# kubernetes-sigs/karpenter

Hardware: AMD Instinct MI355X
Metric: pods scheduled/sec (Solve()) (higher is better)
Workload: dtype int64

## Files before the change

### karpenter_amd/csrc/fast_engine.h

```cpp
#pragma once
#include <type_traits>
#include "kernels.h"
#include "pdq_emul.h"

namespace ks {

constexpr int kFastRows = 4;
constexpr uint32_t kFastFree = 0xFFFFFFFFu;
constexpr uint32_t kFastLastBit = 0x80000000u;
constexpr int kFastEnt = 1024;
constexpr int kFastPool = 256;
constexpr int kFastMaxPareto = 16;
constexpr int kFastMaxVar = 12;
constexpr uint64_t kFastExtBit = 1ull << 63;
constexpr int kFastVarBits = 56;

struct FastClaim { uint64_t vmask; int32_t req[4]; };
template <int R> struct FastRec { uint64_t vmask; int32_t req[4]; uint64_t acc[R]; };
struct FastSlot { uint64_t cvmask; uint64_t dmask; int32_t size[4]; uint32_t tmplok; uint32_t kdef; };
struct FastEnt { uint64_t vmask; int32_t cap[4]; uint32_t info; uint32_t pad; };

struct FastPlan {
  int total_bytes, cap;
  int off_state, off_key, off_ord, off_snap, off_ent, off_pool, off_slot, off_misc, off_hot;
// ... 177 lines not shown
KS_FN KS_LDS T* fast_uniform(KS_LDS T* p) {
  return (KS_LDS T*)(uintptr_t)(uint32_t)__builtin_amdgcn_readfirstlane((int)(uint32_t)(uintptr_t)p);
}
#endif
template <class T>
KS_FN T* fast_uniform(T* p) {
#if KS_DEVICE
  const uint64_t u = (uint64_t)p;
  const uint32_t lo = (uint32_t)__builtin_amdgcn_readfirstlane((int)(uint32_t)u), hi = (uint32_t)__builtin_amdgcn_readfirstlane((int)(uint32_t)(u >> 32));
  return (T*)((uint64_t)lo | ((uint64_t)hi << 32));
#else
  return p;
#endif
}

template <bool H, int R> KS_FN ClaimRecs<H, R> fast_uniform(ClaimRecs<H, R> c) { c.p = fast_uniform(c.p); return c; }

#define KS_LIKELY(x) __builtin_expect(!!(x), 1)
#define KS_UNLIKELY(x) __builtin_expect(!!(x), 0)
#if KS_DEVICE
#define KS_COLD __device__ __attribute__((noinline))
#else
#define KS_COLD inline
#endif

KS_FN uint32_t fast_hash(uint64_t vm) {
  const uint32_t lo = (uint32_t)vm, hi = (uint32_t)(vm >> 32);
  return (((lo ^ ((hi << 15) | (hi >> 17))) * 0x9E3779B1u) >> 22) & (kFastEnt - 1);
}
KS_FN int fast_lookup(const KS_LDS FastEnt* ent, uint64_t vm, FastEnt& out) {
  uint32_t h = fast_hash(vm);
  for (int probe = 0; probe < kFastEnt; ++probe) {
    out = lds_get(&ent[h]);
    if (!(out.info & 1u)) return -1;
    if ((out.vmask & ~kFastExtBit) == vm) return (int)h;
    h = (h + 1) & (kFastEnt - 1);
  }
  return -1;
}
KS_FN bool fast_fits_first(const FastEnt& e, const int32_t* req, const int32_t* size) {
  return (int)(size[0] <= e.cap[0] - req[0]) & (int)(size[1] <= e.cap[1] - req[1]) & (int)(size[2] <= e.cap[2] - req[2]) & (int)(size[3] <= e.cap[3] - req[3]);
}
KS_FN bool fast_fits(const KS_LDS int32_t* pool, const FastEnt& e, const int32_t* req, const int32_t* size) {
  if (fast_fits_first(e, req, size)) return true;
  const int extra = (int)((e.info >> 8) & 0xFFu);
  const int off = (int)(e.info >> 16);
// ... 936 lines not shown
      const KS_LDS FastEnt* en = ent;
      W::for_n(n, [&](int i) { const uint32_t c = oo[i]; go[i] = c; gn[c] = ok_[i]; });
      W::for_n(n, [&](int c) {
        const FastClaim st = ls.state((uint32_t)c);
        FastEnt e;
        gs[c] = st;
        ge[c] = (uint16_t)fast_lookup(en, st.vmask, e);
      });
      W::store(S.n_claims_out, n_claims);
    }
    FastNodes nd{};
    if (F.nodes) nd = *F.nodes;
    if (status == 0 && nd.limit_hit) status = 2;
    if (status) W::store(S.status_out, status);
    Counters c{};
    c.bin_evaluations = n_tests + n_cold_tests + nd.n_tests; c.full_evaluations = n_steps; c.queue_pops = steps + nd.n_placed; c.sorts = steps; c.slow_sorts = order.slow_sorts;
    c.column_resets = (unsigned long long)n_evict; c.ref_bin_evaluations = n_ref + n_ref_extra + nd.n_ref;
    c.decline = (unsigned long long)(bail_code > 0 ? bail_code : 0);
    if (tc) for (int i = 0; i < 16; ++i) c.cycles[i] = tc[i];
#ifdef KSOLVE_PHASE_TIMERS
    for (int i = 0; i < 4; ++i) c.cycles[16 + i] = hs->hw[i];
    c.cycles[20] = t_small | (n_small << 44);
    c.cycles[18] = (hs->hw[2] << 32) | (unsigned long long)(hs->mail.simd[0] | (hs->mail.simd[1] << 8) | (hs->mail.simd[2] << 16) | (hs->mail.simd[3] << 24));
#endif
    if (F.nodes) c.cycles[19] = (unsigned long long)nd.variant;
    if (F.lim) c.full_filters = (unsigned long long)(F.lim->n_ids - (uint32_t)Pk->n_templates) | ((unsigned long long)R << 16) | ((unsigned long long)F.lim->first_claim << 32);
    if (W::leader()) *S.counters = c;
    W::sync();
  }
};

template <int GS, int R>
struct FastHotCtx {
  typename FastMem<GS, R>::o16 okey, oord; typename FastMem<GS, R>::States cst; KS_LDS FastEnt* ent; KS_LDS int32_t* pool;
  KS_LDS FastSlot* aslot; KS_LDS FastHot* hs;
};
enum { FEV_DONE = 0, FEV_REFRESH = 1, FEV_SLOT = 2, FEV_SLOWSORT = 3, FEV_PLACE = 4, FEV_NEWCLAIM = 5, FEV_COUNT = 6, FEV_SLOW = 7, FEV_CONT = 8, FEV_DEAD = 9 };

template <int R>
struct FastHelperK {
  LaneVar<uint32_t> tok[R];
  LaneVar<uint64_t> cvm[R], dm[R], gd[R];
  LaneVar<int32_t> z0[R], z1[R], z2[R], z3[R];
  uint32_t gen = 0xFFFFFFFFu, miss = 0;
};
template <class W, int R>
// ... 82 lines not shown
KS_DEV void fast_helper_run(const FastWork* f, char* lds) {
  const FastPlan& pl = f->plan;
  FastHotCtx<GS, R> cx;
  cx.hs = fast_uniform((KS_LDS FastHot*)(lds + pl.off_hot));
  cx.cst.p = fast_uniform((KS_LDS FastRec<R>*)(lds + pl.off_state));
  cx.okey = nullptr; cx.oord = nullptr;
  cx.ent = fast_uniform((KS_LDS FastEnt*)(lds + pl.off_ent));
  cx.pool = fast_uniform((KS_LDS int32_t*)(lds + pl.off_pool));
  cx.aslot = fast_uniform((KS_LDS FastSlot*)(lds + pl.off_slot));
  KS_LDS FastMail* const mail = &cx.hs->mail;
  FastHelperK<R> k;
  uint32_t seen = 0;
  for (;;) {
    const uint32_t w0 = mail_load(&mail->word[0]), w1 = mail_load(&mail->word[1]), quit = mail_load(&mail->quit);
    if (fast_uniform((int)quit) != 0) break;
    const uint32_t nxt = seen + 1u;
    const uint32_t w = (uint32_t)fast_uniform((int)((nxt & 1u) ? w1 : w0));
    if ((w >> 16) != (nxt & 0xFFFFu)) continue;
    fast_helper_serve<W, GS, R>(k, cx, nxt, w);
    seen = nxt;
  }
}
#endif

template <class W, int GS, int R>
KS_COLD int fast_slow_run(FastHotCtx<GS, R> cx, int budget) {
  budget = fast_uniform(budget);
  typedef typename FastMem<GS, R>::o16 o16;
  const unsigned long long t_in = W::clock();
  const o16 okey = fast_uniform(cx.okey), oord = fast_uniform(cx.oord);
  const typename FastMem<GS, R>::States cst = fast_uniform(cx.cst);
  KS_LDS FastEnt* const ent = fast_uniform(cx.ent);
  KS_LDS int32_t* const pool = fast_uniform(cx.pool);
  KS_LDS FastSlot* const aslot = fast_uniform(cx.aslot);
  KS_LDS FastHot* const hs = fast_uniform(cx.hs);
  const int np = fast_uniform(hs->np), max_steps_in = fast_uniform(hs->max_steps);
  const int max_steps = max_steps_in < 0 ? 0x7FFFFFFF : max_steps_in;
  const KS_GLOBAL uint32_t* const gqcls = (const KS_GLOBAL uint32_t*)fast_uniform(hs->q_class);
  const volatile int* const cancel = fast_uniform(hs->cancel);
  KS_GLOBAL uint32_t* const gqclaim = (KS_GLOBAL uint32_t*)fast_uniform(hs->q_claim);
  KS_GLOBAL uint32_t* const gqcnt = (KS_GLOBAL uint32_t*)fast_uniform(hs->q_cnt);
  int base = fast_uniform(hs->base), bi = fast_uniform(hs->bi), bn = fast_uniform(hs->bn), n = fast_uniform(hs->n), steps = fast_uniform(hs->steps), status = fast_uniform(hs->status);
  int pend_a = fast_uniform(hs->pend_a), pend_x = fast_uniform(hs->pend_x); uint32_t pend_mv = (uint32_t)fast_uniform((int)hs->pend_mv); bool pend_new = fast_uniform(hs->pend_new) != 0;
  unsigned long long n_steps = W::uniform(hs->n_steps), n_ref = W::uniform(hs->n_ref);
  LaneVar<uint32_t> cur[R], scls[R], tok[R], nxt_cls, bcls, oclaim, ocnt;
  LaneVar<uint64_t> cvm[R], dm[R], gd[R];
// ... 23 lines not shown
      if (bn > 0) {
        const int dn = bn, b0 = base;
        W::each([&](int l) { if (l < dn) { gqclaim[b0 + l] = oclaim.at(l); gqcnt[b0 + l] = ocnt.at(l); } });
        base += 64;
      }
      if (base >= np || status) { bn = 0; bi = 0; break; }
      bn = np - base < 64 ? np - base : 64;
      bi = 0;
      const int nb = base + 64;
      W::each([&](int l) { bcls.at(l) = nxt_cls.at(l); });
      W::each([&](int l) { if (nb + l < np) nxt_cls.at(l) = gqcls[nb + l]; });
      if ((base & 1023) == 0 && cancel) {
        const int cv = fast_uniform((int)W::poll_flag(cancel));
        if (cv > 0 || (cv < 0 && base >= -cv)) { status = 2; bn = 0; break; }
      }
    }
    if (KS_UNLIKELY(steps >= max_steps)) { status = 2; break; }
    if (KS_UNLIKELY(pend_a >= 0)) {
      if (pend_new) { ev = FEV_PLACE; break; }
      const int a = pend_a;
      if (!(a + 1 >= n || (uint32_t)okey[a + 1 < n ? a + 1 : a] >= pend_mv) &&
          !(n <= 12 || (n >= 50 && !fast_sampled(n, a)))) { ev = FEV_SLOWSORT; ev_arg = a; break; }
      pend_a = -1;
      int from = a;
      const uint32_t mv = pend_mv;
      for (;;) {
        LaneVar<uint32_t> kv, ov;
        const uint64_t less = W::ballot([&](int l) {
          const int i = from + 1 + l;
          if (i >= n) return false;
          const uint32_t k = okey[i];
          kv.at(l) = k; ov.at(l) = oord[i];
          return k < mv;
        });
        const int s_ = less == ~0ull ? 64 : ctz64(~less);
        if (s_ == 0) break;
        W::each([&](int l) { if (l < s_) { okey[from + l] = (uint16_t)kv.at(l); oord[from + l] = (uint16_t)ov.at(l); } });
        from += s_;
        if (s_ < 64) break;
      }
      if (from != a) {
        if (W::leader()) { okey[from] = (uint16_t)mv; oord[from] = (uint16_t)pend_x; }
        W::sync();
        const int b = from;
        W::each([&](int l) {
#pragma unroll
          for (int j = 0; j < R; ++j) { const uint32_t r = cur[j].at(l); cur[j].at(l) = r - (uint32_t)(((uint32_t)a < r && r <= (uint32_t)b) ? 1 : 0); }
        });
      }
    }
    KS_SEC(ts0)
    const uint32_t clsw = bcls.bcast(bi), kcls = clsw & ~kFastLastBit;
    int row = -1, sl = 0;
    if constexpr (R == 1) {
      const uint64_t m0 = W::ballot([&](int l) { return scls[0].at(l) == kcls; });
      if (KS_LIKELY(m0 != 0)) { row = 0; sl = ctz64(m0); }
    } else {
#pragma unroll
      for (int j = 0; j < R; ++j) {
        const uint64_t mj = W::ballot([&](int l) { return scls[j].at(l) == kcls; });
        if (mj != 0 && row < 0) { row = j; sl = ctz64(mj); }
      }
    }
    if (KS_UNLIKELY(row < 0)) { ev = FEV_SLOT; ev_arg = (int)kcls; break; }
    if constexpr (R == 1) row = 0;
    const int slot = row * 64 + sl;
    const FastSlot cs = lds_get(&aslot[slot]);
// ... 139 lines not shown
      cst.put_state((uint32_t)x, ns);
#pragma unroll
      for (int j = 0; j < R; ++j) cst.put_acc((uint32_t)x, j, accw[j]);
      if (s_ <= 0) okey[a] = (uint16_t)mvn;
      else { okey[a + s_] = (uint16_t)mvn; oord[a + s_] = (uint16_t)x; }
    }
    W::sync();
    KS_SEC(ts3)
    bi++; steps++;
    if (KS_UNLIKELY(cold_refresh)) { ev = FEV_REFRESH; ev_arg = x; break; }
    if (--budget <= 0 && pend_a < 0) { ev = FEV_CONT; break; }
  }
  if (ev == FEV_DONE && bn > 0) {
    const int dn = bi < bn ? bi : bn, b0 = base;
    W::each([&](int l) { if (l < dn) { gqclaim[b0 + l] = oclaim.at(l); gqcnt[b0 + l] = ocnt.at(l); } });
    bn = 0; bi = 0;
  }
  if (W::leader()) {
    hs->base = base; hs->bi = bi; hs->bn = bn; hs->n = n; hs->steps = steps; hs->status = status;
    hs->pend_a = pend_a; hs->pend_x = pend_x; hs->pend_mv = pend_mv; hs->pend_new = pend_new ? 1 : 0;
    hs->n_steps = n_steps; hs->n_ref = n_ref; hs->ev_arg = ev_arg;
    hs->hot_cycles += W::clock() - t_in;
#ifdef KSOLVE_PHASE_TIMERS
    hs->tsec[0] += ts0; hs->tsec[1] += ts1; hs->tsec[2] += ts2; hs->tsec[3] += ts3; hs->tsec[4] += ts4; hs->tsec[5] += ts5; hs->tsec[6] += ts6; hs->tsec[7] += ts7;
#endif
  }
#undef KS_SEC
  W::each([&](int l) {
#pragma unroll
    for (int j = 0; j < R; ++j) { hs->cur[j][l] = cur[j].at(l); hs->scls[j][l] = scls[j].at(l); }
    hs->nxt_cls[l] = nxt_cls.at(l); hs->bcls[l] = bcls.at(l); hs->oclaim[l] = oclaim.at(l); hs->ocnt[l] = ocnt.at(l);
  });
  W::sync();
  return ev;
}

template <class W, int GS, int R, bool HP = false>
KS_COLD int fast_hot_run(FastHotCtx<GS, R> cx) {
  typedef typename FastMem<GS, R>::o16 o16;
  KS_LDS FastHot* const hs = fast_uniform(cx.hs);
  if (fast_uniform(hs->pend_a) >= 0 || fast_uniform(hs->max_steps) >= 0 || fast_uniform(hs->status) != 0 || fast_uniform(hs->n) <= 0) return FEV_SLOW;
  const o16 okey = fast_uniform(cx.okey), oord = fast_uniform(cx.oord);
  const typename FastMem<GS, R>::States cst = fast_uniform(cx.cst);
  KS_LDS FastEnt* const ent = fast_uniform(cx.ent);
  KS_LDS int32_t* const pool = fast_uniform(cx.pool);
  KS_LDS FastSlot* const aslot = fast_uniform(cx.aslot);
  const int np = fast_uniform(hs->np), n = fast_uniform(hs->n);
  const KS_GLOBAL uint32_t* const gqcls = (const KS_GLOBAL uint32_t*)fast_uniform(hs->q_class);
  const bool polled = fast_uniform(hs->cancel) != nullptr;
  KS_GLOBAL uint32_t* const gqclaim = (KS_GLOBAL uint32_t*)fast_uniform(hs->q_claim);
  KS_GLOBAL uint32_t* const gqcnt = (KS_GLOBAL uint32_t*)fast_uniform(hs->q_cnt);
  int base = fast_uniform(hs->base), bi = fast_uniform(hs->bi), bn = fast_uniform(hs->bn), steps = fast_uniform(hs->steps);
  unsigned long long n_ref = W::uniform(hs->n_ref);
  const int bi_in = bi, base_in = base;
  LaneVar<uint32_t> cur[R], scls[R], tok[R], nxt_cls, bcls, oclaim, ocnt;
  LaneVar<uint64_t> cvm[R], dm[R], gd[R];
  LaneVar<int32_t> z0[R], z1[R], z2[R], z3[R];
  W::each([&](int l) {
#pragma unroll
    for (int j = 0; j < R; ++j) {
      cur[j].at(l) = hs->cur[j][l]; scls[j].at(l) = hs->scls[j][l];
      if constexpr (!HP) {
        const FastSlot s = lds_get(&aslot[j * 64 + l]);
// ... 67 lines not shown
  auto stage_a = [&](int i) {
    clsw = bcls.bcast(i & 63);
    const uint32_t kcls = clsw & ~kFastLastBit;
    row = 0;
    if constexpr (R == 1) {
      const uint64_t m0 = W::ballot([&](int l) { return scls[0].at(l) == kcls; });
      slbitA = m0 & (0ull - m0);
      sl = ctz64(m0 | (1ull << 63));
    } else {
      uint64_t mf = 0;
#pragma unroll
      for (int j = R - 1; j >= 0; --j) {
        const uint64_t mj = W::ballot([&](int l) { return scls[j].at(l) == kcls; });
        row = mj != 0 ? j : row; mf = mj != 0 ? mj : mf;
      }
      slbitA = mf & (0ull - mf);
      sl = ctz64(mf | (1ull << 63));
    }
    rc0 = cur[0].bcast(sl);
#pragma unroll
    for (int j = 1; j < R; ++j) { const uint32_t cj = cur[j].bcast(sl); rc0 = row == j ? cj : rc0; }
    order_reads(rc0);
  };
  for (;;) {
    const int bf = bn - ((base + bn >= np || (polled && ((base + 64) & 1023) == 0)) ? 1 : 0);
    if (bi < bf) { stage_a(bi); read_done(); gather(); }
    int bfx = bf;
    while (bi < bfx) {
      uint64_t bad = 0;
      const int slot = row * 64 + sl;
      const FastSlot cs = lds_get(&aslot[slot]);
      const uint64_t slbit = slbitA;
      const int rws = row;
      uint64_t vm = 0;
      auto select = [&]() {
        const int rem = n - (int)rc0;
        vm = rem >= 64 ? ~0ull : ((1ull << (rem < 0 ? 0 : rem)) - 1ull);
        return W::ballot([&](int l) { return (awv.at(l) & slbit) != 0; }) & vm;
      };
      uint64_t okm = select();
      if constexpr (HP) {
        const int x0 = (int)xv.bcast(ctz64(okm | (1ull << 63)));
        if (KS_UNLIKELY((okm != 0) & ((x0 == pend1) | (x0 == pend2)))) {
          const uint32_t dn = (uint32_t)fast_uniform((int)dwl.bcast(0)) >> 1;
          const bool stale1 = pend1 >= 0 && (int32_t)(dn - seq) < 0, stale2 = pend2 >= 0 && (int32_t)(dn - (seq - 1u)) < 0;
          if ((x0 == pend1 && stale1) || (x0 == pend2 && stale2)) {
#ifdef KSOLVE_PHASE_TIMERS
            const unsigned long long tw0 = W::clock();
#endif
            const uint32_t c1 = (uint32_t)(pend1 < 0 ? 0 : pend1), c2 = (uint32_t)(pend2 < 0 ? 0 : pend2);
            uint64_t a1 = 0, a2 = 0;
            uint32_t dw2 = 0;
#if KS_DEVICE
            for (uint32_t spins = 0;; ++spins) {
              const uint32_t dv = mail_load(&mail->done);
              W::order();
              const uint64_t v1 = cst.acc(c1, 0), v2 = cst.acc(c2, 0);
              dw2 = (uint32_t)fast_uniform((int)dv); a1 = W::uniform(v1); a2 = W::uniform(v2);
              if ((int32_t)((dw2 >> 1) - seq) >= 0) break;
              if (spins > (1u << 22)) { dead = true; break; }
// ... 28 lines not shown
#pragma unroll
          for (int j = 0; j < 4; ++j) {
            const int rj = r + 64 * j;
            m4[j] = W::ballot([&](int l) { return ((cst.acc(x4[j].at(l), rws) & slbit) != 0) & (rj + l < n); });
          }
          n_ext++;
#pragma unroll
          for (int j = 3; j >= 0; --j) found = m4[j] != 0 ? r + 64 * j : found;
          r += 256;
        }
        if (found >= 0) {
          rc0 = (uint32_t)found;
          order_reads(rc0);
          gather();
          okm = select();
        }
      }
      const int first_ok = ctz64(okm | (1ull << 63));
      const int a = (int)rc0 + first_ok;
      const int x = (int)xv.bcast(first_ok);
      const uint32_t cnt = kv.bcast(first_ok);
      bad |= cnt >= 65534u ? ~0ull : 0ull;
      FastClaim ns;
      LaneVar<uint64_t> nmv; LaneVar<int32_t> n0v, n1v, n2v, n3v;
      W::each([&](int l) {
        nmv.at(l) = mvv.at(l) & cs.cvmask;
        n0v.at(l) = q0.at(l) + cs.size[0]; n1v.at(l) = q1.at(l) + cs.size[1]; n2v.at(l) = q2.at(l) + cs.size[2]; n3v.at(l) = q3.at(l) + cs.size[3];
      });
      ns.vmask = nmv.bcast(first_ok);
      ns.req[0] = n0v.bcast(first_ok); ns.req[1] = n1v.bcast(first_ok); ns.req[2] = n2v.bcast(first_ok); ns.req[3] = n3v.bcast(first_ok);
      const uint32_t mvn = cnt + 1;
      const uint64_t lessm = W::ballot([&](int l) { return kv.at(l) < mvn; }) & vm;
      const uint64_t tsh = (lessm >> 1) >> first_ok;
      const int sm = ctz64(~tsh);
      bad |= first_ok + 1 + sm >= 64 ? ~0ull : 0ull;
      {
        const uint32_t d1 = (uint32_t)a - e1, d2 = (uint32_t)a - e2, d3 = (uint32_t)a - e3;
        const uint32_t dmin = fast_umin_s(fast_umin_s(d1, d2), d3);
        bad |= ((sm != 0) & (inexact_b | (dmin <= 2u))) ? ~0ull : 0ull;
      }
      if (KS_UNLIKELY(bad != 0)) { bfx = bi; continue; }
      if constexpr (HP) {
        static_assert(!HP || R == 1, "the two-wavefront loop: one row of class slots");
        {
          const uint32_t dw = (uint32_t)fast_uniform((int)dwl.bcast(0));
          if (KS_UNLIKELY(((int32_t)((dw >> 1) - (seq - 1u)) < 0) | ((dw & 1u) != 0))) {
            const uint32_t dw2 = wait_for(seq - 1u);
#ifdef KSOLVE_PHASE_TIMERS
            hw2++;
#endif
            if ((dw2 & 1u) | (uint32_t)dead) break;
          }
        }
        ++seq;
        const int fo = first_ok; const uint32_t sq = seq;
        W::each([&](int l) {
          if (l == fo) {
            FastClaim mine;
            mine.vmask = nmv.at(l); mine.req[0] = n0v.at(l); mine.req[1] = n1v.at(l); mine.req[2] = n2v.at(l); mine.req[3] = n3v.at(l);
            cst.put_state(xv.at(l), mine);
            W::order();
            mail_store(&mail->word[sq & 1u], (sq << 16) | xv.at(l));
          }
        });
        pend2 = pend1; pend1 = x;
#ifdef KSOLVE_PHASE_TIMERS
        t_post = W::clock();
#endif
#if !KS_DEVICE
        if (fast_emu_helper_eager()) wait_for(seq);
#endif
        {
          const int rb = (int)rc0, smv = sm;
          W::each([&](int l) {
            if (l >= fo && l <= fo + smv) {
              const bool me = l == fo;
              const int dst = me ? rb + l + smv : rb + l - 1;
              okey[dst] = (uint16_t)(me ? kv.at(l) + 1u : kv.at(l)); oord[dst] = (uint16_t)xv.at(l);
            }
          });
        }
        W::order();
// ... 36 lines not shown
            okey[dst] = (uint16_t)(me ? kv.at(l) + 1u : kv.at(l)); oord[dst] = (uint16_t)xv.at(l);
          }
        });
      }
      {
        const uint32_t ua1 = (uint32_t)a + 1u, su = (uint32_t)sm;
        const uint32_t lastm = (uint32_t)((int32_t)clsw >> 31);
        const int bb = bi;
        W::each([&](int l) {
          const bool mine = l == bb;
          oclaim.at(l) = mine ? (uint32_t)x : oclaim.at(l); ocnt.at(l) = mine ? cnt : ocnt.at(l);
#pragma unroll
          for (int j = 0; j < R; ++j) {
            const bool me = j * 64 + l == slot;
            const uint32_t fm = me ? lastm : 0u;
            const uint32_t rr = cur[j].at(l);
            cur[j].at(l) = me ? (uint32_t)a : rr - (uint32_t)((rr - ua1) < su);
            scls[j].at(l) |= fm; tok[j].at(l) &= ~fm;
          }
        });
      }
      n_ref += (unsigned long long)((uint32_t)a + 1u);
      const uint32_t tbit = 1u << (uint32_t)(ns.vmask >> 56);
      LaneVar<uint64_t> mlv[R], evm[R];
      LaneVar<int32_t> c0[R], c1[R], c2[R], c3[R];
      uint64_t rowm[R];
      if constexpr (R > 1) {
        W::each([&](int l) {
#pragma unroll
          for (int j = 0; j < R; ++j) mlv[j].at(l) = ns.vmask & cvm[j].at(l);
        });
#pragma unroll
        for (int j = 0; j < R; ++j)
          rowm[j] = W::ballot([&](int l) { return (tok[j].at(l) & tbit) != 0; }) &
                    W::ballot([&](int l) { return (((mlv[j].at(l) & dm[j].at(l)) + dm[j].at(l)) & gd[j].at(l)) == gd[j].at(l); });
      } else rowm[0] = ~0ull;
      W::each([&](int l) {
#pragma unroll
        for (int j = 0; j < R; ++j) {
          if (R > 1 && rowm[j] == 0) continue;
          const uint64_t m = ns.vmask & cvm[j].at(l);
          const FastEnt e = ent_live(&ent[fast_hash(m)]);
          mlv[j].at(l) = m; evm[j].at(l) = e.vmask;
          c0[j].at(l) = e.cap[0]; c1[j].at(l) = e.cap[1]; c2[j].at(l) = e.cap[2]; c3[j].at(l) = e.cap[3];
        }
      });
      const int fo_ = first_ok;
      LaneVar<uint32_t> xw;
      W::each([&](int l) { xw.at(l) = xv.at(l); });
      if constexpr (FastMem<GS, R>::kOrderHbm) W::hbm_sync(); else W::order();
      W::sched_fence();
      stage_a(bi + 1);
      W::sched_fence();
      uint64_t accw[R];
#pragma unroll
      for (int j = 0; j < R; ++j) {
        if (R > 1 && rowm[j] == 0) { accw[j] = 0; continue; }
        const uint64_t tokm = R > 1 ? rowm[j] : W::ballot([&](int l) { return (tok[j].at(l) & tbit) != 0; });
        const uint64_t fldm = R > 1 ? ~0ull : W::ballot([&](int l) { return (((mlv[j].at(l) & dm[j].at(l)) + dm[j].at(l)) & gd[j].at(l)) == gd[j].at(l); });
        const uint64_t simm = W::ballot([&](int l) { return evm[j].at(l) == mlv[j].at(l); });
        const uint64_t f0 = W::ballot([&](int l) { return z0[j].at(l) <= c0[j].at(l) - ns.req[0]; });
        const uint64_t f1 = W::ballot([&](int l) { return z1[j].at(l) <= c1[j].at(l) - ns.req[1]; });
        const uint64_t f2 = W::ballot([&](int l) { return z2[j].at(l) <= c2[j].at(l) - ns.req[2]; });
        const uint64_t f3 = W::ballot([&](int l) { return z3[j].at(l) <= c3[j].at(l) - ns.req[3]; });
        const uint64_t basem = tokm & fldm, fitm = f0 & f1 & f2 & f3;
        uint64_t accm = basem & simm & fitm;
        const uint64_t oddm = basem & ~simm;
        if (KS_UNLIKELY(oddm != 0)) {
          uint64_t ok2 = 0, missm = 0;
          W::ballot2([&](int l) {
            if (!((oddm >> l) & 1)) return 0;
            FastEnt e;
            if (fast_lookup(ent, mlv[j].at(l), e) < 0) return 2;
            const int32_t sz[4] = {z0[j].at(l), z1[j].at(l), z2[j].at(l), z3[j].at(l)};
            return fast_fits(pool, e, ns.req, sz) ? 1 : 0;
          }, ok2, missm);
          accm |= ok2;
          if (missm) { rf = x; bfx = bi + 1; }
        }
        accw[j] = accm;
      }
      W::each([&](int l) {
        if (l == fo_) {
          FastRec<R> mine;
          mine.vmask = nmv.at(l); mine.req[0] = n0v.at(l); mine.req[1] = n1v.at(l); mine.req[2] = n2v.at(l); mine.req[3] = n3v.at(l);
#pragma unroll
          for (int j = 0; j < R; ++j) mine.acc[j] = accw[j];
          cst.put_rec(xw.at(l), mine);
        }
      });
      if constexpr (FastMem<GS, R>::kStateHbm) W::hbm_sync(); else W::order();
      gather();
      bi++; steps++;
    }
    if (bi < bf || bf < bn || rf >= 0) break;
    if (bn > 0) {
      const int dn = bn, b0 = base;
      W::each([&](int l) { if (l < dn) { gqclaim[b0 + l] = oclaim.at(l); gqcnt[b0 + l] = ocnt.at(l); } });
    }
    const int nbase = bn > 0 ? base + 64 : base;
    if (nbase >= np || (polled && (nbase & 1023) == 0)) break;
    base = nbase;
    bn = np - base < 64 ? np - base : 64;
    bi = 0;
    const int nb = base + 64;
    W::each([&](int l) { bcls.at(l) = nxt_cls.at(l); });
    W::each([&](int l) { if (nb + l < np) nxt_cls.at(l) = gqcls[nb + l]; });
  }
  int rf2 = -1;
  if constexpr (HP) {
    const uint32_t dw = wait_for(seq);
    if (KS_UNLIKELY((dw & 1u) != 0)) {
      rf = fast_uniform((int)mail->miss_x[0]); rf2 = fast_uniform((int)mail->miss_x[1]);
      if (rf < 0) { rf = rf2; rf2 = -1; }
      W::order();
      if (W::leader()) { mail->miss_x[0] = -1; mail->miss_x[1] = -1; mail_store(&mail->done, seq << 1); }
      W::order();
    }
    if (KS_UNLIKELY(dead)) return FEV_DEAD;
#ifdef KSOLVE_PHASE_TIMERS
    if (W::leader()) { hs->hw[0] += hw0; hs->hw[1] += hw1; hs->hw[2] += hw2; hs->hw[3] += hw3; }
#endif
  }
  if (bi != bi_in || base != base_in) {
    if (W::leader()) { hs->base = base; hs->bi = bi; hs->bn = bn; hs->steps = steps; hs->n_ref = n_ref; hs->rf_x = rf; hs->rf_x2 = rf2; hs->n_steps += 4 * n_ext; }
    W::each([&](int l) {
#pragma unroll
      for (int j = 0; j < R; ++j) { hs->cur[j][l] = cur[j].at(l); hs->scls[j][l] = scls[j].at(l); }
      hs->nxt_cls[l] = nxt_cls.at(l); hs->bcls[l] = bcls.at(l); hs->oclaim[l] = oclaim.at(l); hs->ocnt[l] = ocnt.at(l);
    });
    W::sync();
  }
  return FEV_SLOW;
}

template <class W, int GS = 0, int R = 1, bool HP = false, bool US = kFastKeepBuiltIn, bool PO = kFastKeepBuiltIn>
struct FastEngine {
  FastCold<W, GS, R, US, PO> cold;
  KS_LDS FastHot* hs;
  KS_DEV FastEngine(const ProblemView* p, const Workspace* s, const FastWork* f, char* lds) { cold.init(p, s, f, lds); hs = cold.hs; }

  KS_DEV void solve() {
    KS_LDS FastHot* const h = fast_uniform(hs);
    W::each([&](int l) { for (int j = 0; j < kFastRows; ++j) { h->cur[j][l] = 0; h->scls[j][l] = kFastFree; } });
    W::sync();
    {
      const int why = (int)W::uniform((uint64_t)(uint32_t)cold.setup());
      if (why) { cold.bail_code = why; cold.finish(3, 0, 0, 0, 0, 0, nullptr); return; }
    }
    const FastNodes* const nds = fast_uniform(cold.Fk->nodes);
    if (nds && fast_uniform((int)nds->bail) != 0) { cold.bail_code = fast_uniform((int)nds->bail); cold.finish(3, 0, 0, 0, 0, 0, nullptr); return; }
    const int np = nds ? fast_uniform((int)nds->n_left) : fast_uniform(cold.Pk->n_pods);
    if (W::leader()) {
      h->base = 0; h->bi = 0; h->bn = 0; h->n = 0; h->np = np; h->steps = 0; h->status = 0;
      const long long ms_ = cold.Sk->max_steps;
      h->max_steps = ms_ < 0 ? -1 : (nds || ms_ > 0x7FFFFFFF) ? 0x7FFFFFFF : (int)ms_;
      h->pend_a = -1; h->pend_x = 0; h->pend_mv = 0; h->pend_new = 0; h->ev_arg = 0; h->rf_x = -1; h->rf_x2 = -1;
      h->n_steps = 0; h->n_tests = 0; h->n_ref = 0; h->hot_cycles = 0;
      for (int i = 0; i < 8; ++i) h->tsec[i] = 0;
      for (int i = 0; i < 4; ++i) h->hw[i] = 0;
      h->q_class = cold.Fk->q_class; h->cancel = cold.Sk->cancel_flag;
      h->q_claim = cold.Fk->q_claim; h->q_cnt = cold.Fk->q_cnt;
    }
    {
      const uint32_t* qc = cold.Fk->q_class;
      W::each([&](int l) { h->nxt_cls[l] = l < np ? qc[l] : 0; h->bcls[l] = 0; h->oclaim[l] = 0; h->ocnt[l] = 0; });
    }
    W::sync();
    FastHotCtx<GS, R> cx;
    cx.okey = cold.order.key; cx.oord = cold.order.ord; cx.cst = cold.cst; cx.ent = cold.ent; cx.pool = cold.pool;
    cx.aslot = cold.aslot; cx.hs = hs;
    unsigned long long tev[8] = {0, 0, 0, 0, 0, 0, 0, 0}, nev[8] = {0, 0, 0, 0, 0, 0, 0, 0};
    unsigned long long t_fast = 0, n_fast = 0, t_slow = 0, n_slow = 0;
    const unsigned long long t_begin = W::clock();
    const bool use_fast = fast_uniform(h->max_steps) < 0;
    for (;;) {
      const unsigned long long tf0 = W::clock();
      const bool place_now = use_fast && fast_uniform(h->pend_new) != 0 && fast_uniform(h->bi) < fast_uniform(h->bn) && fast_uniform(h->status) == 0;
      int ev = place_now ? (int)FEV_PLACE : use_fast ? fast_uniform(fast_hot_run<W, GS, R, HP>(cx)) : (int)FEV_SLOW;
      t_fast += W::clock() - tf0; n_fast++;
      if (HP && ev == FEV_DEAD) { cold.bail_code = DECLINE_REFRESHER_DEAD; cold.finish(3, 0, 0, 0, 0, 0, nullptr); return; }
      if (use_fast && fast_uniform(h->rf_x) >= 0) {
        const int rx = fast_uniform(h->rf_x), rx2 = HP ? fast_uniform(h->rf_x2) : -1;
        if (W::leader()) { h->rf_x = -1; h->rf_x2 = -1; }
        W::sync();
        if (fast_uniform(cold.refresh_claim(rx)) < 0) { cold.bail_code = DECLINE_REFRESH_FAILED; cold.finish(3, 0, 0, 0, 0, 0, nullptr); return; }
        if (rx2 >= 0 && fast_uniform(cold.refresh_claim(rx2)) < 0) { cold.bail_code = DECLINE_REFRESH_FAILED; cold.finish(3, 0, 0, 0, 0, 0, nullptr); return; }
        continue;
      }
      if (ev == FEV_SLOW) { const unsigned long long ts0 = W::clock(); ev = fast_uniform(fast_slow_run<W, GS, R>(cx, use_fast ? 1 : 0x7FFFFFFF)); t_slow += W::clock() - ts0; n_slow++; }
      if (ev == FEV_CONT) continue;
      if (ev == FEV_DONE) break;
      const unsigned long long te0 = W::clock();
      if (ev == FEV_REFRESH) {
        if (fast_uniform(cold.refresh_claim(fast_uniform(h->ev_arg))) < 0) { cold.bail_code = DECLINE_REFRESH_FAILED; cold.finish(3, 0, 0, 0, 0, 0, nullptr); return; }
      } else if (ev == FEV_SLOT) {
        if (fast_uniform(cold.new_slot(fast_uniform(h->ev_arg))) < 0) { cold.finish(3, 0, 0, 0, 0, 0, nullptr); return; }
      } else if (ev == FEV_SLOWSORT || ev == FEV_PLACE) {
        const int n = fast_uniform(h->n);
        int b = -1;
        if (ev == FEV_SLOWSORT) cold.slow_sort(n, fast_uniform(h->ev_arg), 0);
        else b = fast_uniform(cold.place_new_claim(n));
// ... 136 lines not shown
```

### karpenter_amd/host/ksched.cpp

```cpp
#include <dlfcn.h>
#include <pthread.h>

#include <algorithm>
#include <climits>
#include <chrono>
#include <condition_variable>
#include <mutex>
#include <cstring>
#include <functional>
#include <map>
#include <unordered_map>
#include <set>
#include <stdexcept>
#include <string>
#include <thread>
#include <vector>

#include "../../include/ksolve.h"
#include "../csrc/engine_setting.h"
#include "../csrc/reqalg.h"
#include "json_mini.hpp"

namespace ks {
inline ReqRef reqbuf_ref_with_minv(const ReqBuf& b) { ReqRef r = b.ref(); r.minv = b.minv; return r; }
// ... 2509 lines not shown
        t.set("classify_ms", Value::number(api.kernel_ms(handle, "classify")));
        t.set("row_hash_ms", Value::number(api.kernel_ms(handle, "row_hash")));
        t.set("sort_ms", Value::number(api.kernel_ms(handle, "sort")));
        t.set("it_index_ms", Value::number(api.kernel_ms(handle, "it_index")));
      }
      timings.push(t);
    }

    Value out = Value::object();
    auto uid_of = [&](int p) { if (!uid_text[p].empty()) return uid_text[p]; std::string s; uint64_t a, b; group_uid(group_of_pod[p].first, group_of_pod[p].second, a, b, &s); return s; };
    const ksolve_claims& cl = res.claims;
    Value counters = Value::object();
    counters.set("binEvaluations", Value::integer((int64_t)res.bin_evaluations));
    counters.set("instanceTypeEvaluations", Value::integer((int64_t)res.it_evaluations));
    counters.set("referenceBinEvaluations", Value::integer((int64_t)res.ref_bin_evaluations));
    counters.set("pops", Value::integer((int64_t)res.queue_pops)); counters.set("sorts", Value::integer((int64_t)res.sorts));
    counters.set("slowSorts", Value::integer((int64_t)res.slow_sorts)); counters.set("relaxations", Value::integer((int64_t)res.relaxations));
    counters.set("pods", Value::integer(own->base ? own->probe_pods : n_pods)); counters.set("claims", Value::integer(cl.n_claims));
    counters.set("engine", Value::string(res.engine_used == 2 ? "cursor" : res.engine_used == 3 ? "spread" : "general")); counters.set("cursorClaimStateInHBM", Value::boolean(res.engine_used == 2 && res.cursor_wide != 0)); counters.set("cursorMemoryPlan", Value::integer(res.engine_used == 2 ? (int64_t)res.cursor_wide : -1)); counters.set("cursorAttempts", Value::integer((int64_t)res.cursor_attempts)); counters.set("engineFallbackReason", Value::integer((int64_t)res.engine_fallback_reason));
    counters.set("rows", Value::integer(n_rows)); counters.set("instanceTypes", Value::integer(n_its)); counters.set("strictTableShared", Value::boolean(S->strict_shared));
    counters.set("topologyGroups", Value::integer(S->n_topo_groups)); counters.set("topologyAliasClasses", Value::integer(S->n_alias_classes));
    counters.set("reqWords", Value::integer(rw)); counters.set("itWords", Value::integer(it_words)); counters.set("keys", Value::integer(nk)); counters.set("resources", Value::integer(n_res));
    { Value pc = Value::array(); for (int i = 0; i < 24; ++i) pc.push(Value::integer((int64_t)res.phase_cycles[i])); counters.set("phaseCycles", pc); }
    out.set("counters", counters);
    out.set("timings", timings);
    out.set("timedOut", Value::boolean(st == KSOLVE_ERR_CANCELLED));
    out.set("packingCost", Value::number(res.packing_cost));
    {
      auto pvec = (decltype(&ksolve_packing_vector))dlsym(api.lib, "ksolve_packing_vector");
      if (pvec && st == KSOLVE_OK) {
        std::vector<double> cnt(n_its), cst(n_its);
        if (pvec(handle, &res, cnt.data(), cst.data()) == KSOLVE_OK) {
          Value pv = Value::array();
          for (int i = 0; i < n_its; ++i) if (cnt[i] > 0) { Value e = Value::array(); e.push(Value::integer(i)); e.push(Value::number(cnt[i])); e.push(Value::number(cst[i])); pv.push(e); }
          out.set("packingVector", pv);
        }
      }
    }
    int unscheduled = 0;
    for (int p = 0; p < n_pods; ++p) if (in_probe(p) && res.pod_assignment[p] == -1) unscheduled++;
    { int64_t there = 0; for (size_t e = 0; e < S->node_names.size(); ++e) if (node_there(e)) there++; counters.set("existingNodes", Value::integer(there)); }
    out.set("scheduledPods", Value::integer((own->base ? own->probe_pods : n_pods) - unscheduled));
    if (want_results) {
      std::vector<std::vector<std::pair<uint32_t, int>>> members(want_results == 1 ? cl.n_claims : 0);
      std::vector<uint32_t> member_count(cl.n_claims, 0);
      std::vector<std::vector<std::pair<uint32_t, int>>> node_members(S->node_names.size());
// ... 341 lines not shown
```

Measured before the change: 1.602 million.

## Handle the stopping pod inside the hot loop instead of returning to the slow path

When the fast hot loop stops partway through a batch, it now finishes that one pod itself. It places the claim, refreshes the fit records, does the stable key move and returns a specific event (new claim, slot, slow sort or continue) instead of always handing control to the slow path. The aim is to cut the round trips between the hot and cold routines and the state reload each one costs. Shared helpers (claim_add, refresh_reads/words, put_record, fast_stable_move) are factored out to support this. The change adds more code and register pressure to the hot kernel, adds new correctness-sensitive bookkeeping for pending moves and step counters, and adds phase-timer counters.

```diff
diff --git a/karpenter_amd/csrc/fast_engine.h b/karpenter_amd/csrc/fast_engine.h
--- a/karpenter_amd/csrc/fast_engine.h
+++ b/karpenter_amd/csrc/fast_engine.h
@@ -223,6 +223,9 @@
 #define KS_COLD __device__ __attribute__((noinline))
 #else
 #define KS_COLD inline
+#endif
+#ifndef KSOLVE_LOOP_TAIL
+#define KSOLVE_LOOP_TAIL 15
 #endif
 
 KS_FN uint32_t fast_hash(uint64_t vm) {
@@ -1205,6 +1208,10 @@
     for (int i = 0; i < 4; ++i) c.cycles[16 + i] = hs->hw[i];
     c.cycles[20] = t_small | (n_small << 44);
     c.cycles[18] = (hs->hw[2] << 32) | (unsigned long long)(hs->mail.simd[0] | (hs->mail.simd[1] << 8) | (hs->mail.simd[2] << 16) | (hs->mail.simd[3] << 24));
+    if (tc && !(hs->hw[0] | hs->hw[1] | hs->hw[2] | hs->hw[3])) {
+      c.cycles[16] = hs->tsec[0] | (hs->tsec[1] << 32); c.cycles[17] = hs->tsec[2] | (hs->tsec[3] << 32);
+      c.cycles[7] = hs->tsec[4]; c.cycles[18] = hs->tsec[5]; c.cycles[19] = hs->tsec[6];
+    }
 #endif
     if (F.nodes) c.cycles[19] = (unsigned long long)nd.variant;
     if (F.lim) c.full_filters = (unsigned long long)(F.lim->n_ids - (uint32_t)Pk->n_templates) | ((unsigned long long)R << 16) | ((unsigned long long)F.lim->first_claim << 32);
@@ -1333,6 +1340,31 @@
   }
 }
 #endif
+
+template <class W, class O16>
+KS_FN int fast_stable_move(O16 okey, O16 oord, int n, int a, uint32_t mv, int x) {
+  int from = a;
+  for (;;) {
+    LaneVar<uint32_t> kv, ov;
+    const uint64_t less = W::ballot([&](int l) {
+      const int i = from + 1 + l;
+      if (i >= n) return false;
+      const uint32_t k = okey[i];
+      kv.at(l) = k; ov.at(l) = oord[i];
+      return k < mv;
+    });
+    const int s_ = less == ~0ull ? 64 : ctz64(~less);
+    if (s_ == 0) break;
+    W::each([&](int l) { if (l < s_) { okey[from + l] = (uint16_t)kv.at(l); oord[from + l] = (uint16_t)ov.at(l); } });
+    from += s_;
+    if (s_ < 64) break;
+  }
+  if (from != a) {
+    if (W::leader()) { okey[from] = (uint16_t)mv; oord[from] = (uint16_t)x; }
+    W::sync();
+  }
+  return from;
+}
 
 template <class W, int GS, int R>
 KS_COLD int fast_slow_run(FastHotCtx<GS, R> cx, int budget) {
@@ -1402,27 +1434,8 @@
       if (!(a + 1 >= n || (uint32_t)okey[a + 1 < n ? a + 1 : a] >= pend_mv) &&
           !(n <= 12 || (n >= 50 && !fast_sampled(n, a)))) { ev = FEV_SLOWSORT; ev_arg = a; break; }
       pend_a = -1;
-      int from = a;
-      const uint32_t mv = pend_mv;
-      for (;;) {
-        LaneVar<uint32_t> kv, ov;
-        const uint64_t less = W::ballot([&](int l) {
-          const int i = from + 1 + l;
-          if (i >= n) return false;
-          const uint32_t k = okey[i];
-          kv.at(l) = k; ov.at(l) = oord[i];
-          return k < mv;
-        });
-        const int s_ = less == ~0ull ? 64 : ctz64(~less);
-        if (s_ == 0) break;
-        W::each([&](int l) { if (l < s_) { okey[from + l] = (uint16_t)kv.at(l); oord[from + l] = (uint16_t)ov.at(l); } });
-        from += s_;
-        if (s_ < 64) break;
-      }
-      if (from != a) {
-        if (W::leader()) { okey[from] = (uint16_t)mv; oord[from] = (uint16_t)pend_x; }
-        W::sync();
-        const int b = from;
+      const int b = fast_stable_move<W>(okey, oord, n, a, pend_mv, pend_x);
+      if (b != a) {
         W::each([&](int l) {
 #pragma unroll
           for (int j = 0; j < R; ++j) { const uint32_t r = cur[j].at(l); cur[j].at(l) = r - (uint32_t)(((uint32_t)a < r && r <= (uint32_t)b) ? 1 : 0); }
@@ -1608,7 +1621,7 @@
     hs->n_steps = n_steps; hs->n_ref = n_ref; hs->ev_arg = ev_arg;
     hs->hot_cycles += W::clock() - t_in;
 #ifdef KSOLVE_PHASE_TIMERS
-    hs->tsec[0] += ts0; hs->tsec[1] += ts1; hs->tsec[2] += ts2; hs->tsec[3] += ts3; hs->tsec[4] += ts4; hs->tsec[5] += ts5; hs->tsec[6] += ts6; hs->tsec[7] += ts7;
+    hs->tsec[0] += ts0; hs->tsec[1] += ts1; hs->tsec[2] += ts2; hs->tsec[3] += ts3;
 #endif
   }
 #undef KS_SEC
@@ -1622,9 +1635,13 @@
 }
 
 template <class W, int GS, int R, bool HP = false>
-KS_COLD int fast_hot_run(FastHotCtx<GS, R> cx) {
+KS_COLD int fast_hot_run(FastHotCtx<GS, R> cx, int behind_first) {
   typedef typename FastMem<GS, R>::o16 o16;
   KS_LDS FastHot* const hs = fast_uniform(cx.hs);
+  behind_first = fast_uniform(behind_first);
+#ifdef KSOLVE_PHASE_TIMERS
+  if (fast_uniform(hs->pend_a) >= 0 && fast_uniform(hs->max_steps) < 0 && fast_uniform(hs->status) == 0 && W::leader()) hs->tsec[6] += 1ull;
+#endif
   if (fast_uniform(hs->pend_a) >= 0 || fast_uniform(hs->max_steps) >= 0 || fast_uniform(hs->status) != 0 || fast_uniform(hs->n) <= 0) return FEV_SLOW;
   const o16 okey = fast_uniform(cx.okey), oord = fast_uniform(cx.oord);
   const typename FastMem<GS, R>::States cst = fast_uniform(cx.cst);
@@ -1738,6 +1755,86 @@
     for (int j = 1; j < R; ++j) { const uint32_t cj = cur[j].bcast(sl); rc0 = row == j ? cj : rc0; }
     order_reads(rc0);
   };
+  auto window_mask = [&]() -> uint64_t {
+    const int rem = n - (int)rc0;
+    return rem >= 64 ? ~0ull : ((1ull << (rem < 0 ? 0 : rem)) - 1ull);
+  };
+  struct AddRegs { LaneVar<uint64_t> nmv; LaneVar<int32_t> n0v, n1v, n2v, n3v; };
+  auto claim_add = [&](const FastSlot& cs, int fo, AddRegs& s, FastClaim& ns) {
+    W::each([&](int l) {
+      s.nmv.at(l) = mvv.at(l) & cs.cvmask;
+      s.n0v.at(l) = q0.at(l) + cs.size[0]; s.n1v.at(l) = q1.at(l) + cs.size[1]; s.n2v.at(l) = q2.at(l) + cs.size[2]; s.n3v.at(l) = q3.at(l) + cs.size[3];
+    });
+    ns.vmask = s.nmv.bcast(fo);
+    ns.req[0] = s.n0v.bcast(fo); ns.req[1] = s.n1v.bcast(fo); ns.req[2] = s.n2v.bcast(fo); ns.req[3] = s.n3v.bcast(fo);
+  };
+  struct RefreshRegs { LaneVar<uint64_t> mlv[R], evm[R]; LaneVar<int32_t> c0[R], c1[R], c2[R], c3[R]; uint64_t rowm[R]; };
+  auto refresh_reads = [&](const FastClaim& ns, uint32_t tbit, RefreshRegs& g) {
+    if constexpr (R > 1) {
+      W::each([&](int l) {
+#pragma unroll
+        for (int j = 0; j < R; ++j) g.mlv[j].at(l) = ns.vmask & cvm[j].at(l);
+      });
+#pragma unroll
+      for (int j = 0; j < R; ++j)
+        g.rowm[j] = W::ballot([&](int l) { return (tok[j].at(l) & tbit) != 0; }) &
+                    W::ballot([&](int l) { return (((g.mlv[j].at(l) & dm[j].at(l)) + dm[j].at(l)) & gd[j].at(l)) == gd[j].at(l); });
+    } else g.rowm[0] = ~0ull;
+    W::each([&](int l) {
+#pragma unroll
+      for (int j = 0; j < R; ++j) {
+        if (R > 1 && g.rowm[j] == 0) continue;
+        const uint64_t m = ns.vmask & cvm[j].at(l);
+        const FastEnt e = ent_live(&ent[fast_hash(m)]);
+        g.mlv[j].at(l) = m; g.evm[j].at(l) = e.vmask;
+        g.c0[j].at(l) = e.cap[0]; g.c1[j].at(l) = e.cap[1]; g.c2[j].at(l) = e.cap[2]; g.c3[j].at(l) = e.cap[3];
+      }
+    });
+  };
+  auto refresh_words = [&](const FastClaim& ns, uint32_t tbit, RefreshRegs& g, uint64_t (&accw)[R], auto&& on_miss) {
+#pragma unroll
+    for (int j = 0; j < R; ++j) {
+      if (R > 1 && g.rowm[j] == 0) { accw[j] = 0; continue; }
+      const uint64_t tokm = R > 1 ? g.rowm[j] : W::ballot([&](int l) { return (tok[j].at(l) & tbit) != 0; });
+      const uint64_t fldm = R > 1 ? ~0ull : W::ballot([&](int l) { return (((g.mlv[j].at(l) & dm[j].at(l)) + dm[j].at(l)) & gd[j].at(l)) == gd[j].at(l); });
+      const uint64_t simm = W::ballot([&](int l) { return g.evm[j].at(l) == g.mlv[j].at(l); });
+      const uint64_t f0 = W::ballot([&](int l) { return z0[j].at(l) <= g.c0[j].at(l) - ns.req[0]; });
+      const uint64_t f1 = W::ballot([&](int l) { return z1[j].at(l) <= g.c1[j].at(l) - ns.req[1]; });
+      const uint64_t f2 = W::ballot([&](int l) { return z2[j].at(l) <= g.c2[j].at(l) - ns.req[2]; });
+      const uint64_t f3 = W::ballot([&](int l) { return z3[j].at(l) <= g.c3[j].at(l) - ns.req[3]; });
+      const uint64_t basem = tokm & fldm, fitm = f0 & f1 & f2 & f3;
+      uint64_t accm = basem & simm & fitm;
+      const uint64_t oddm = basem & ~simm;
+      if (KS_UNLIKELY(oddm != 0)) {
+        uint64_t ok2 = 0, missm = 0;
+        W::ballot2([&](int l) {
+          if (!((oddm >> l) & 1)) return 0;
+          FastEnt e;
+          if (fast_lookup(ent, g.mlv[j].at(l), e) < 0) return 2;
+          const int32_t sz[4] = {z0[j].at(l), z1[j].at(l), z2[j].at(l), z3[j].at(l)};
+          return fast_fits(pool, e, ns.req, sz) ? 1 : 0;
+        }, ok2, missm);
+        accm |= ok2;
+        if (missm) on_miss();
+      }
+      accw[j] = accm;
+    }
+  };
+  auto put_record = [&](int fo, LaneVar<uint32_t>& xw, AddRegs& s, const uint64_t (&accw)[R]) {
+    W::each([&](int l) {
+      if (l == fo) {
+        FastRec<R> mine;
+        mine.vmask = s.nmv.at(l); mine.req[0] = s.n0v.at(l); mine.req[1] = s.n1v.at(l); mine.req[2] = s.n2v.at(l); mine.req[3] = s.n3v.at(l);
+#pragma unroll
+        for (int j = 0; j < R; ++j) mine.acc[j] = accw[j];
+        cst.put_rec(xw.at(l), mine);
+      }
+    });
+  };
+  bool stopped = false;
+#ifdef KSOLVE_PHASE_TIMERS
+  auto count_exit = [&](int why) { if (W::leader()) hs->tsec[4 + why / 3] += 1ull << (21 * (why % 3)); };
+#endif
   for (;;) {
     const int bf = bn - ((base + bn >= np || (polled && ((base + 64) & 1023) == 0)) ? 1 : 0);
     if (bi < bf) { stage_a(bi); read_done(); gather(); }
@@ -1750,8 +1847,7 @@
       const int rws = row;
       uint64_t vm = 0;
       auto select = [&]() {
-        const int rem = n - (int)rc0;
-        vm = rem >= 64 ? ~0ull : ((1ull << (rem < 0 ? 0 : rem)) - 1ull);
+        vm = window_mask();
         return W::ballot([&](int l) { return (awv.at(l) & slbit) != 0; }) & vm;
       };
       uint64_t okm = select();
@@ -1826,13 +1922,8 @@
       const uint32_t cnt = kv.bcast(first_ok);
       bad |= cnt >= 65534u ? ~0ull : 0ull;
       FastClaim ns;
-      LaneVar<uint64_t> nmv; LaneVar<int32_t> n0v, n1v, n2v, n3v;
-      W::each([&](int l) {
-        nmv.at(l) = mvv.at(l) & cs.cvmask;
-        n0v.at(l) = q0.at(l) + cs.size[0]; n1v.at(l) = q1.at(l) + cs.size[1]; n2v.at(l) = q2.at(l) + cs.size[2]; n3v.at(l) = q3.at(l) + cs.size[3];
-      });
-      ns.vmask = nmv.bcast(first_ok);
-      ns.req[0] = n0v.bcast(first_ok); ns.req[1] = n1v.bcast(first_ok); ns.req[2] = n2v.bcast(first_ok); ns.req[3] = n3v.bcast(first_ok);
+      AddRegs nsv;
+      claim_add(cs, first_ok, nsv, ns);
       const uint32_t mvn = cnt + 1;
       const uint64_t lessm = W::ballot([&](int l) { return kv.at(l) < mvn; }) & vm;
       const uint64_t tsh = (lessm >> 1) >> first_ok;
@@ -1861,7 +1952,7 @@
         W::each([&](int l) {
           if (l == fo) {
             FastClaim mine;
-            mine.vmask = nmv.at(l); mine.req[0] = n0v.at(l); mine.req[1] = n1v.at(l); mine.req[2] = n2v.at(l); mine.req[3] = n3v.at(l);
+            mine.vmask = nsv.nmv.at(l); mine.req[0] = nsv.n0v.at(l); mine.req[1] = nsv.n1v.at(l); mine.req[2] = nsv.n2v.at(l); mine.req[3] = nsv.n3v.at(l);
             cst.put_state(xv.at(l), mine);
             W::order();
             mail_store(&mail->word[sq & 1u], (sq << 16) | xv.at(l));
@@ -1944,29 +2035,8 @@
       }
       n_ref += (unsigned long long)((uint32_t)a + 1u);
       const uint32_t tbit = 1u << (uint32_t)(ns.vmask >> 56);
-      LaneVar<uint64_t> mlv[R], evm[R];
-      LaneVar<int32_t> c0[R], c1[R], c2[R], c3[R];
-      uint64_t rowm[R];
-      if constexpr (R > 1) {
-        W::each([&](int l) {
-#pragma unroll
-          for (int j = 0; j < R; ++j) mlv[j].at(l) = ns.vmask & cvm[j].at(l);
-        });
-#pragma unroll
-        for (int j = 0; j < R; ++j)
-          rowm[j] = W::ballot([&](int l) { return (tok[j].at(l) & tbit) != 0; }) &
-                    W::ballot([&](int l) { return (((mlv[j].at(l) & dm[j].at(l)) + dm[j].at(l)) & gd[j].at(l)) == gd[j].at(l); });
-      } else rowm[0] = ~0ull;
-      W::each([&](int l) {
-#pragma unroll
-        for (int j = 0; j < R; ++j) {
-          if (R > 1 && rowm[j] == 0) continue;
-          const uint64_t m = ns.vmask & cvm[j].at(l);
-          const FastEnt e = ent_live(&ent[fast_hash(m)]);
-          mlv[j].at(l) = m; evm[j].at(l) = e.vmask;
-          c0[j].at(l) = e.cap[0]; c1[j].at(l) = e.cap[1]; c2[j].at(l) = e.cap[2]; c3[j].at(l) = e.cap[3];
-        }
-      });
+      RefreshRegs rg;
+      refresh_reads(ns, tbit, rg);
       const int fo_ = first_ok;
       LaneVar<uint32_t> xw;
       W::each([&](int l) { xw.at(l) = xv.at(l); });
@@ -1975,52 +2045,24 @@
       stage_a(bi + 1);
       W::sched_fence();
       uint64_t accw[R];
-#pragma unroll
-      for (int j = 0; j < R; ++j) {
-        if (R > 1 && rowm[j] == 0) { accw[j] = 0; continue; }
-        const uint64_t tokm = R > 1 ? rowm[j] : W::ballot([&](int l) { return (tok[j].at(l) & tbit) != 0; });
-        const uint64_t fldm = R > 1 ? ~0ull : W::ballot([&](int l) { return (((mlv[j].at(l) & dm[j].at(l)) + dm[j].at(l)) & gd[j].at(l)) == gd[j].at(l); });
-        const uint64_t simm = W::ballot([&](int l) { return evm[j].at(l) == mlv[j].at(l); });
-        const uint64_t f0 = W::ballot([&](int l) { return z0[j].at(l) <= c0[j].at(l) - ns.req[0]; });
-        const uint64_t f1 = W::ballot([&](int l) { return z1[j].at(l) <= c1[j].at(l) - ns.req[1]; });
-        const uint64_t f2 = W::ballot([&](int l) { return z2[j].at(l) <= c2[j].at(l) - ns.req[2]; });
-        const uint64_t f3 = W::ballot([&](int l) { return z3[j].at(l) <= c3[j].at(l) - ns.req[3]; });
-        const uint64_t basem = tokm & fldm, fitm = f0 & f1 & f2 & f3;
-        uint64_t accm = basem & simm & fitm;
-        const uint64_t oddm = basem & ~simm;
-        if (KS_UNLIKELY(oddm != 0)) {
-          uint64_t ok2 = 0, missm = 0;
-          W::ballot2([&](int l) {
-            if (!((oddm >> l) & 1)) return 0;
-            FastEnt e;
-            if (fast_lookup(ent, mlv[j].at(l), e) < 0) return 2;
-            const int32_t sz[4] = {z0[j].at(l), z1[j].at(l), z2[j].at(l), z3[j].at(l)};
-            return fast_fits(pool, e, ns.req, sz) ? 1 : 0;
-          }, ok2, missm);
-          accm |= ok2;
-          if (missm) { rf = x; bfx = bi + 1; }
-        }
-        accw[j] = accm;
-      }
-      W::each([&](int l) {
-        if (l == fo_) {
-          FastRec<R> mine;
-          mine.vmask = nmv.at(l); mine.req[0] = n0v.at(l); mine.req[1] = n1v.at(l); mine.req[2] = n2v.at(l); mine.req[3] = n3v.at(l);
-#pragma unroll
-          for (int j = 0; j < R; ++j) mine.acc[j] = accw[j];
-          cst.put_rec(xw.at(l), mine);
-        }
-      });
+      refresh_words(ns, tbit, rg, accw, [&]() { rf = x; bfx = bi + 1; });
+      put_record(fo_, xw, nsv, accw);
       if constexpr (FastMem<GS, R>::kStateHbm) W::hbm_sync(); else W::order();
       gather();
       bi++; steps++;
     }
-    if (bi < bf || bf < bn || rf >= 0) break;
+#ifdef KSOLVE_PHASE_TIMERS
+    if (rf >= 0) count_exit(7); else if (bi >= bf && bf < bn) count_exit(base + bn >= np ? 5 : 4);
+#endif
+    if (bi < bf || bf < bn || rf >= 0) { stopped = bi < bf && rf < 0; break; }
     if (bn > 0) {
       const int dn = bn, b0 = base;
       W::each([&](int l) { if (l < dn) { gqclaim[b0 + l] = oclaim.at(l); gqcnt[b0 + l] = ocnt.at(l); } });
     }
     const int nbase = bn > 0 ? base + 64 : base;
+#ifdef KSOLVE_PHASE_TIMERS
+    if (nbase >= np || (polled && (nbase & 1023) == 0)) count_exit(nbase >= np ? 5 : 4);
+#endif
     if (nbase >= np || (polled && (nbase & 1023) == 0)) break;
     base = nbase;
     bn = np - base < 64 ? np - base : 64;
@@ -2028,6 +2070,108 @@
     const int nb = base + 64;
     W::each([&](int l) { bcls.at(l) = nxt_cls.at(l); });
     W::each([&](int l) { if (nb + l < np) nxt_cls.at(l) = gqcls[nb + l]; });
+  }
+  int ev = FEV_SLOW, ev_arg = 0;
+  int pa = -1, px = 0; uint32_t pmv = 0;
+  unsigned long long n_more = 0;
+  const bool placed = behind_first == 2 ? (bi != 0 || base != base_in + 64)
+                                        : (bi != bi_in || base != base_in) && !(behind_first == 1 && bi == bi_in + 1 && base == base_in);
+  if constexpr (!HP) if (stopped) {
+    const int slot = row * 64 + sl;
+    const uint64_t slbit = slbitA;
+    const uint64_t vm = window_mask();
+    const uint64_t okm = W::ballot([&](int l) { return (awv.at(l) & slbit) != 0; }) & vm;
+    uint32_t cur0 = cur[0].bcast(sl);
+#pragma unroll
+    for (int j = 1; j < R; ++j) { const uint32_t cj = cur[j].bcast(sl); cur0 = row == j ? cj : cur0; }
+    const uint32_t lastm = (uint32_t)((int32_t)clsw >> 31);
+    const int first_ok = ctz64(okm | (1ull << 63));
+    const int a = (int)rc0 + first_ok;
+    const int x = (int)xv.bcast(first_ok);
+    const uint32_t cnt = kv.bcast(first_ok);
+    const uint32_t mvn = cnt + 1;
+    const uint64_t lessm = W::ballot([&](int l) { return kv.at(l) < mvn; }) & vm;
+    const int sm = ctz64(~((lessm >> 1) >> first_ok));
+    const bool reach = first_ok + 1 + sm >= 64;
+#ifdef KSOLVE_PHASE_TIMERS
+    count_exit(slbit == 0 ? 3 : okm == 0 ? 1 : cnt >= 65534u ? 8 : reach ? 2 : 0);
+#endif
+    if (okm == 0) {
+      if ((KSOLVE_LOOP_TAIL & 2) != 0 && slbit != 0) {
+        const bool inside = (int)cur0 < n;
+        const uint32_t nr = inside ? (uint32_t)n : cur0;
+        n_more = inside ? (unsigned long long)((n - (int)cur0 + 63) / 64 - 1) : 0ull;
+        W::each([&](int l) {
+#pragma unroll
+          for (int j = 0; j < R; ++j) {
+            const bool me = j * 64 + l == slot;
+            cur[j].at(l) = me ? nr : cur[j].at(l);
+            scls[j].at(l) |= me ? lastm : 0u;
+          }
+        });
+        steps++;
+        ev = FEV_NEWCLAIM; ev_arg = slot;
+      } else if ((KSOLVE_LOOP_TAIL & 4) != 0 && slbit == 0) {
+        ev = FEV_SLOT; ev_arg = (int)(clsw & ~kFastLastBit);
+      }
+    } else if ((KSOLVE_LOOP_TAIL & (reach ? 8 : 1)) != 0 && cnt < 65534u) {
+      const FastSlot cs = lds_get(&aslot[slot]);
+      FastClaim ns;
+      AddRegs nsv;
+      claim_add(cs, first_ok, nsv, ns);
+      {
+        const int bb = bi;
+        W::each([&](int l) {
+          const bool mine = l == bb;
+          oclaim.at(l) = mine ? (uint32_t)x : oclaim.at(l); ocnt.at(l) = mine ? cnt : ocnt.at(l);
+#pragma unroll
+          for (int j = 0; j < R; ++j) {
+            const bool me = j * 64 + l == slot;
+            const uint32_t fm = me ? lastm : 0u;
+            cur[j].at(l) = me ? (uint32_t)a : cur[j].at(l);
+            scls[j].at(l) |= fm; tok[j].at(l) &= ~fm;
+          }
+        });
+      }
+      n_ref += (unsigned long long)((uint32_t)a + 1u);
+      n_more = (unsigned long long)(((uint32_t)a - cur0) >> 6);
+      const uint32_t tbit = 1u << (uint32_t)(ns.vmask >> 56);
+      RefreshRegs rg;
+      refresh_reads(ns, tbit, rg);
+      uint64_t accw[R];
+      refresh_words(ns, tbit, rg, accw, [&]() { rf = x; });
+      {
+        const int rb = (int)rc0, fo = first_ok;
+        W::each([&](int l) { if (l == fo) okey[rb + l] = (uint16_t)(kv.at(l) + 1u); });
+      }
+      put_record(first_ok, xv, nsv, accw);
+      if constexpr (FastMem<GS, R>::kOrderHbm || FastMem<GS, R>::kStateHbm) W::hbm_sync();
+      bi++; steps++;
+      pa = a; px = x; pmv = mvn;
+      if (rf < 0) {
+        W::sync();
+        const bool movable = a + 1 < n && (uint32_t)okey[a + 1 < n ? a + 1 : a] < mvn;
+        if (movable && !(n <= 12 || (n >= 50 && !fast_sampled(n, a)))) { ev = FEV_SLOWSORT; ev_arg = a; }
+        else {
+          const int b = movable ? fast_stable_move<W>(okey, oord, n, a, mvn, x) : a;
+          if (b != a) {
+            W::each([&](int l) {
+#pragma unroll
+              for (int j = 0; j < R; ++j) { const uint32_t r = cur[j].at(l); cur[j].at(l) = r - (uint32_t)(((uint32_t)a < r && r <= (uint32_t)b) ? 1 : 0); }
+            });
+          }
+          pa = -1;
+          if (bi < bn) {
+            stage_a(bi);
+            if (slbitA == 0) { if ((KSOLVE_LOOP_TAIL & 4) != 0) { ev = FEV_SLOT; ev_arg = (int)(clsw & ~kFastLastBit); } }
+            else if (bi < bn - ((base + bn >= np || (polled && ((base + 64) & 1023) == 0)) ? 1 : 0) && bi + 1 < bn) {
+              gather();
+              if ((W::ballot([&](int l) { return (awv.at(l) & slbitA) != 0; }) & window_mask()) != 0) ev = FEV_CONT;
+            }
+          }
+        }
+      }
+    }
   }
   int rf2 = -1;
   if constexpr (HP) {
@@ -2044,16 +2188,23 @@
     if (W::leader()) { hs->hw[0] += hw0; hs->hw[1] += hw1; hs->hw[2] += hw2; hs->hw[3] += hw3; }
 #endif
   }
-  if (bi != bi_in || base != base_in) {
-    if (W::leader()) { hs->base = base; hs->bi = bi; hs->bn = bn; hs->steps = steps; hs->n_ref = n_ref; hs->rf_x = rf; hs->rf_x2 = rf2; hs->n_steps += 4 * n_ext; }
+  if (bi != bi_in || base != base_in || ev == FEV_NEWCLAIM) {
+    if (W::leader()) {
+      hs->base = base; hs->bi = bi; hs->bn = bn; hs->steps = steps; hs->n_ref = n_ref; hs->rf_x = rf; hs->rf_x2 = rf2; hs->n_steps += (placed ? 4 * n_ext : 0ull) + n_more;
+      if (pa >= 0) { hs->pend_a = pa; hs->pend_x = px; hs->pend_mv = pmv; }
+      hs->ev_arg = ev_arg;
+    }
     W::each([&](int l) {
 #pragma unroll
       for (int j = 0; j < R; ++j) { hs->cur[j][l] = cur[j].at(l); hs->scls[j][l] = scls[j].at(l); }
       hs->nxt_cls[l] = nxt_cls.at(l); hs->bcls[l] = bcls.at(l); hs->oclaim[l] = oclaim.at(l); hs->ocnt[l] = ocnt.at(l);
     });
     W::sync();
-  }
-  return FEV_SLOW;
+  } else if (ev != FEV_SLOW) {
+    if (W::leader()) hs->ev_arg = ev_arg;
+    W::sync();
+  }
+  return ev;
 }
 
 template <class W, int GS = 0, int R = 1, bool HP = false, bool US = kFastKeepBuiltIn, bool PO = kFastKeepBuiltIn>
@@ -2096,10 +2247,12 @@
     unsigned long long t_fast = 0, n_fast = 0, t_slow = 0, n_slow = 0;
     const unsigned long long t_begin = W::clock();
     const bool use_fast = fast_uniform(h->max_steps) < 0;
+    int behind_first = 0;
     for (;;) {
       const unsigned long long tf0 = W::clock();
       const bool place_now = use_fast && fast_uniform(h->pend_new) != 0 && fast_uniform(h->bi) < fast_uniform(h->bn) && fast_uniform(h->status) == 0;
-      int ev = place_now ? (int)FEV_PLACE : use_fast ? fast_uniform(fast_hot_run<W, GS, R, HP>(cx)) : (int)FEV_SLOW;
+      int ev = place_now ? (int)FEV_PLACE : use_fast ? fast_uniform(fast_hot_run<W, GS, R, HP>(cx, behind_first)) : (int)FEV_SLOW;
+      behind_first = !(use_fast && !place_now) ? 0 : ev == FEV_CONT ? 1 : (ev == FEV_SLOWSORT && fast_uniform(h->bi) >= fast_uniform(h->bn)) ? 2 : 0;
       t_fast += W::clock() - tf0; n_fast++;
       if (HP && ev == FEV_DEAD) { cold.bail_code = DECLINE_REFRESHER_DEAD; cold.finish(3, 0, 0, 0, 0, 0, nullptr); return; }
       if (use_fast && fast_uniform(h->rf_x) >= 0) {
diff --git a/karpenter_amd/host/ksched.cpp b/karpenter_amd/host/ksched.cpp
--- a/karpenter_amd/host/ksched.cpp
+++ b/karpenter_amd/host/ksched.cpp
@@ -2555,6 +2555,7 @@
     counters.set("topologyGroups", Value::integer(S->n_topo_groups)); counters.set("topologyAliasClasses", Value::integer(S->n_alias_classes));
     counters.set("reqWords", Value::integer(rw)); counters.set("itWords", Value::integer(it_words)); counters.set("keys", Value::integer(nk)); counters.set("resources", Value::integer(n_res));
     { Value pc = Value::array(); for (int i = 0; i < 24; ++i) pc.push(Value::integer((int64_t)res.phase_cycles[i])); counters.set("phaseCycles", pc); }
+    if (res.engine_used == 2) counters.set("onePodLoopCalls", Value::integer((int64_t)res.phase_cycles[11]));
     out.set("counters", counters);
     out.set("timings", timings);
     out.set("timedOut", Value::boolean(st == KSOLVE_ERR_CANCELLED));
```

New measurement: 1.629 million (median of 6 runs). +1.7%, better.
